# Chemical118/TREW

Hardware: AMD Instinct MI355X
Metric: Gbases/s scanned (short 5 32, 150 bp reads) (higher is better)
Workload: dtype u32

## Files before the change

include/trew_hip.h:

```cpp
#ifndef TREW_HIP_H
#define TREW_HIP_H

#include <stddef.h>
#include <stdint.h>

#ifdef __cplusplus
extern "C" {
#endif

#define TREW_HIP_ABI_VERSION 4

enum {
    TREW_MODE_SHORT = 0,
    TREW_MODE_PAIR = 1,
    TREW_MODE_LONG = 2,
    TREW_MODE_SEGMENT = 3
};

enum {
    TREW_TABLE_FORWARD_HIGH = 0,
    TREW_TABLE_FORWARD_LOW = 1,
    TREW_TABLE_BACKWARD_HIGH = 2,
    TREW_TABLE_BACKWARD_LOW = 3,
    TREW_TABLE_BOTH_HIGH = 4,
    TREW_TABLE_BOTH_LOW = 5,
    TREW_NUM_TABLES = 6
};

enum {
    TREW_FLAG_NO_FILTER = 1,
    TREW_FLAG_DEBUG_NO_EMIT = 2,
    TREW_FLAG_DEBUG_NO_KLOOP = 4,
    TREW_FLAG_DEBUG_POISON_LDS = 32,
    TREW_FLAG_DEBUG_WIDE_NO_WAIT = 128,
    TREW_FLAG_NO_TIMING = 64,
    TREW_FLAG_COMPAT_G1 = 512,
    TREW_FLAG_DEBUG_NO_JOINT = 2048,
    TREW_FLAG_DEBUG_NO_GROUP = 1024,
    TREW_FLAG_TRACK_PRESSURE = 256
};

typedef struct {
    int32_t min_mer;
    int32_t max_mer;
    double low_baseline;
    double high_baseline;
    int32_t slice_length;
    int32_t mode;
    int32_t device;
    int32_t n_slots;
    uint64_t max_batch_words;
    uint64_t max_batch_reads;
    uint32_t table_log2_slots;
    uint32_t flags;
    uint64_t max_batch_ascii_bytes;
} trew_hip_params;

typedef struct {
    const uint32_t *words;
    uint64_t n_words;
    const uint32_t *offsets;
    const uint32_t *lengths;
    uint32_t uniform_length;
    uint32_t uniform_stride;
    uint64_t n_reads;
    int32_t on_device;
    int32_t max_length;
} trew_hip_batch;

typedef struct {
    const char *bases;
    uint64_t n_bytes;
    const uint32_t *byte_offsets;
    const uint32_t *lengths;
    const uint32_t *word_offsets;
    uint32_t uniform_length;
    uint32_t reserved;
    uint64_t n_reads;
} trew_hip_ascii_batch;

typedef struct {
    int32_t k;
    int32_t table;
    uint64_t word_lo;
    uint64_t word_hi;
    uint64_t count;
} trew_hip_row;

typedef struct trew_hip_ctx trew_hip_ctx;

int trew_hip_init(const trew_hip_params *params, trew_hip_ctx **out);
void trew_hip_destroy(trew_hip_ctx *ctx);
const char *trew_hip_last_error(const trew_hip_ctx *ctx);

int trew_hip_submit(trew_hip_ctx *ctx, const trew_hip_batch *batch, int slot);
int trew_hip_submit_ascii(trew_hip_ctx *ctx, const trew_hip_ascii_batch *batch, int slot);
int trew_hip_pack_ascii(trew_hip_ctx *ctx, const trew_hip_ascii_batch *batch, uint32_t *words, uint64_t words_cap, uint64_t *n_words);
int trew_hip_wait(trew_hip_ctx *ctx, int slot);

int trew_hip_collect(trew_hip_ctx *ctx, int table, trew_hip_row *rows, uint64_t cap, uint64_t *n_rows);
int trew_hip_reset_tables(trew_hip_ctx *ctx);
int trew_hip_add_rows(trew_hip_ctx *ctx, const trew_hip_row *rows, uint64_t n_rows);

int trew_hip_collect_device(trew_hip_ctx *ctx, trew_hip_row *d_rows, uint64_t cap, uint64_t *n_rows);
int trew_hip_add_rows_device(trew_hip_ctx *ctx, const trew_hip_row *d_rows, uint64_t n_rows);
int trew_hip_merge(trew_hip_ctx *dst, trew_hip_ctx *src);
int trew_hip_add_gathered_device(trew_hip_ctx *ctx, const trew_hip_row *d_buf, uint32_t n_slices, uint32_t own_slice,
                                 uint64_t slice_rows, void *producer_stream, uint64_t *max_rows);
int trew_hip_collect_slice_device(trew_hip_ctx *ctx, trew_hip_row *d_slice, uint64_t slice_rows, void *consumer_stream, uint64_t *n_rows);

int trew_hip_table_pressure(trew_hip_ctx *ctx, uint64_t *used_slots, uint64_t *total_slots, uint64_t *spilled_rows,
                            uint64_t *spill_capacity);

#define TREW_DEBUG_COUNTERS 8
int trew_hip_debug_counters(trew_hip_ctx *ctx, uint64_t *out, int n);

int trew_hip_debug_worklist(trew_hip_ctx *ctx, int slot, uint32_t *units, uint64_t cap, uint64_t *n);

int trew_hip_segment_results(trew_hip_ctx *ctx, int slot, int32_t *k_high, int32_t *k_low,
                             uint64_t *seq_high, uint64_t *seq_low, uint64_t *seq_high_hi, uint64_t *seq_low_hi,
                             uint64_t n_reads);
int trew_hip_filter_masks(trew_hip_ctx *ctx, const trew_hip_batch *batch, uint64_t *cand, int slots_per_read);

int trew_hip_last_timing(trew_hip_ctx *ctx, int slot, float *ms_filter, float *ms_exact, uint64_t *n_flagged);

uint64_t trew_pack_words(uint64_t n_bases);
uint64_t trew_pack_reads(const char *buf, const int64_t *st, const int64_t *nd, uint64_t n_reads,
                         uint32_t *words, uint64_t words_cap, uint32_t *offsets, uint32_t *lengths);

uint64_t trew_pack_pairs(const char *buf1, const int64_t *st1, const int64_t *nd1,
                         const char *buf2, const int64_t *st2, const int64_t *nd2, uint64_t n_pairs,
                         uint32_t *words, uint64_t words_cap, uint32_t *offsets, uint32_t *lengths);

int trew_synth_short_ascii(uint64_t seed, uint64_t first_read, uint64_t n_reads, uint32_t read_len, char *out);
int trew_synth_short_device(trew_hip_ctx *ctx, uint64_t seed, uint64_t first_read, uint64_t n_reads,
                            uint32_t read_len, uint32_t *d_words);
int trew_synth_pair_ascii(uint64_t seed, uint64_t first_pair, uint64_t n_pairs, uint32_t read_len, char *out1, char *out2);
int trew_synth_pair_device(trew_hip_ctx *ctx, uint64_t seed, uint64_t first_pair, uint64_t n_pairs,
                           uint32_t read_len, uint32_t *d_words);

int trew_synth_long_lengths(uint64_t seed, uint64_t first_read, uint64_t n_reads, uint32_t *lengths);
int trew_synth_long_ascii(uint64_t seed, uint64_t first_read, uint64_t n_reads, const uint64_t *byte_offsets, char *out);
int trew_synth_long_device(trew_hip_ctx *ctx, uint64_t seed, uint64_t first_read, uint64_t n_reads,
                           const uint32_t *d_offsets, uint32_t *d_words);

int trew_hip_malloc(trew_hip_ctx *ctx, uint64_t bytes, void **d_ptr);
int trew_hip_free(trew_hip_ctx *ctx, void *d_ptr);
int trew_hip_memcpy_h2d(trew_hip_ctx *ctx, void *d_dst, const void *h_src, uint64_t bytes);
int trew_hip_memcpy_d2h(trew_hip_ctx *ctx, void *h_dst, const void *d_src, uint64_t bytes);
int trew_hip_host_alloc(trew_hip_ctx *ctx, uint64_t bytes, void **h_ptr);
int trew_hip_host_free(trew_hip_ctx *ctx, void *h_ptr);
int trew_hip_device_count(void);
int trew_hip_abi_version(void);

#ifdef __cplusplus
}
#endif
#endif
```

trew_amd/__init__.py:

```python
from . import capi
from .capi import (
    FLAG_NO_FILTER,
    FLAG_DEBUG_POISON_LDS,
    FLAG_NO_TIMING,
    FLAG_TRACK_PRESSURE,
    FLAG_COMPAT_G1,
    FLAG_DEBUG_NO_GROUP,
    FLAG_DEBUG_NO_JOINT,
    FLAG_DEBUG_WIDE_NO_WAIT,
    MODE_LONG,
    MODE_PAIR,
    MODE_SEGMENT,
    MODE_SHORT,
    TABLE_NAMES,
    TrewHip,
    TrewHipError,
    k_mer_check,
    pack_reads,
)
```

trew_amd/capi.py:

```python
from __future__ import annotations

import ctypes as C
import os

import numpy as np

_HERE = os.path.dirname(os.path.abspath(__file__))
LIB_PATH = os.environ.get("TREW_HIP_LIB") or os.path.join(_HERE, "lib", "libtrew_hip.so")

MODE_SHORT, MODE_PAIR, MODE_LONG, MODE_SEGMENT = 0, 1, 2, 3
FLAG_NO_FILTER = 1
FLAG_DEBUG_POISON_LDS = 32
FLAG_NO_TIMING = 64
FLAG_COMPAT_G1 = 512
FLAG_TRACK_PRESSURE = 256
FLAG_DEBUG_NO_JOINT = 2048
FLAG_DEBUG_NO_GROUP = 1024
FLAG_DEBUG_WIDE_NO_WAIT = 128
TABLE_NAMES = ("forward_high", "forward_low", "backward_high", "backward_low", "both_high", "both_low")

EXPORTED_SYMBOLS = (
    "trew_hip_init", "trew_hip_destroy", "trew_hip_last_error", "trew_hip_submit", "trew_hip_wait",
    "trew_hip_collect", "trew_hip_reset_tables", "trew_hip_add_rows", "trew_hip_segment_results",
    "trew_hip_filter_masks", "trew_hip_last_timing", "trew_pack_words", "trew_pack_reads",
    "trew_synth_short_ascii", "trew_synth_short_device", "trew_synth_pair_ascii", "trew_synth_pair_device",
    "trew_hip_malloc", "trew_hip_free", "trew_hip_memcpy_h2d", "trew_hip_memcpy_d2h", "trew_hip_abi_version",
    "trew_pack_pairs", "trew_hip_host_alloc", "trew_hip_host_free", "trew_hip_device_count",
    "trew_synth_long_lengths", "trew_synth_long_ascii", "trew_synth_long_device",
    "trew_hip_collect_device", "trew_hip_add_rows_device", "trew_hip_merge", "trew_hip_table_pressure",
    "trew_hip_add_gathered_device", "trew_hip_collect_slice_device", "trew_hip_debug_counters", "trew_hip_debug_worklist", "trew_hip_submit_ascii", "trew_hip_pack_ascii",
)
DEBUG_COUNTERS = ("strict_rerun", "windows_fallback", "wide_spin_timeout", "inserted", "inserted_wide", "group_punt", "group_routed", "group_target")


class Params(C.Structure):
    _fields_ = [
        ("min_mer", C.c_int32), ("max_mer", C.c_int32),
        ("low_baseline", C.c_double), ("high_baseline", C.c_double),
        ("slice_length", C.c_int32), ("mode", C.c_int32), ("device", C.c_int32), ("n_slots", C.c_int32),
        ("max_batch_words", C.c_uint64), ("max_batch_reads", C.c_uint64),
        ("table_log2_slots", C.c_uint32), ("flags", C.c_uint32),
        ("max_batch_ascii_bytes", C.c_uint64),
    ]


class Batch(C.Structure):
    _fields_ = [
        ("words", C.c_void_p), ("n_words", C.c_uint64),
        ("offsets", C.c_void_p), ("lengths", C.c_void_p),
        ("uniform_length", C.c_uint32), ("uniform_stride", C.c_uint32),
        ("n_reads", C.c_uint64), ("on_device", C.c_int32), ("max_length", C.c_int32),
    ]


class AsciiBatch(C.Structure):
    _fields_ = [
        ("bases", C.c_void_p), ("n_bytes", C.c_uint64),
        ("byte_offsets", C.c_void_p), ("lengths", C.c_void_p), ("word_offsets", C.c_void_p),
        ("uniform_length", C.c_uint32), ("reserved", C.c_uint32), ("n_reads", C.c_uint64),
    ]


class Row(C.Structure):
    _fields_ = [("k", C.c_int32), ("table", C.c_int32), ("word_lo", C.c_uint64), ("word_hi", C.c_uint64),
                ("count", C.c_uint64)]


ROW_DTYPE = np.dtype([("k", "<i4"), ("table", "<i4"), ("word_lo", "<u8"), ("word_hi", "<u8"), ("count", "<u8")])
assert ROW_DTYPE.itemsize == C.sizeof(Row)

_lib = None


def rows_to_tables(rows):
    out = {name: {} for name in TABLE_NAMES}
    if len(rows) == 0:
        return out
    for t, k, lo, hi, c in zip(rows["table"].tolist(), rows["k"].tolist(), rows["word_lo"].tolist(),
                               rows["word_hi"].tolist(), rows["count"].tolist()):
        out[TABLE_NAMES[t]][(k, (hi << 64) | lo)] = c
    return out


def tables_to_rows(tables):
    items = [(k, t, w & 0xFFFFFFFFFFFFFFFF, w >> 64, c)
             for t, name in enumerate(TABLE_NAMES) for (k, w), c in tables.get(name, {}).items()]
    return np.array(items, dtype=ROW_DTYPE) if items else np.zeros(0, dtype=ROW_DTYPE)


def load():
    global _lib
    if _lib is not None:
        return _lib
    if not os.path.exists(LIB_PATH):
        raise OSError("libtrew_hip.so is not built: run `python -c 'import __graft_entry__ as g; g.build()'`")
    lib = C.CDLL(LIB_PATH)
    vp, u64, i32 = C.c_void_p, C.c_uint64, C.c_int
    lib.trew_hip_abi_version.restype = i32
    lib.trew_hip_init.argtypes = [C.POINTER(Params), C.POINTER(vp)]
    lib.trew_hip_destroy.argtypes = [vp]
    lib.trew_hip_destroy.restype = None
    lib.trew_hip_last_error.argtypes = [vp]
    lib.trew_hip_last_error.restype = C.c_char_p
    lib.trew_hip_submit.argtypes = [vp, C.POINTER(Batch), i32]
    lib.trew_hip_wait.argtypes = [vp, i32]
    lib.trew_hip_submit_ascii.argtypes = [vp, C.POINTER(AsciiBatch), i32]
    lib.trew_hip_pack_ascii.argtypes = [vp, C.POINTER(AsciiBatch), vp, u64, C.POINTER(u64)]
    lib.trew_hip_collect.argtypes = [vp, i32, C.POINTER(Row), u64, C.POINTER(u64)]
    lib.trew_hip_reset_tables.argtypes = [vp]
    lib.trew_hip_add_rows.argtypes = [vp, C.POINTER(Row), u64]
    lib.trew_hip_collect_device.argtypes = [vp, vp, u64, C.POINTER(u64)]
    lib.trew_hip_add_rows_device.argtypes = [vp, vp, u64]
    lib.trew_hip_merge.argtypes = [vp, vp]
    lib.trew_hip_add_gathered_device.argtypes = [vp, vp, C.c_uint32, C.c_uint32, u64, vp, C.POINTER(u64)]
    lib.trew_hip_collect_slice_device.argtypes = [vp, vp, u64, vp, C.POINTER(u64)]
    lib.trew_hip_debug_counters.argtypes = [vp, C.POINTER(u64), i32]
    lib.trew_hip_debug_worklist.argtypes = [vp, i32, vp, u64, C.POINTER(u64)]
    lib.trew_hip_table_pressure.argtypes = [vp, C.POINTER(u64), C.POINTER(u64), C.POINTER(u64), C.POINTER(u64)]
    lib.trew_hip_segment_results.argtypes = [vp, i32, vp, vp, vp, vp, vp, vp, u64]
    lib.trew_hip_filter_masks.argtypes = [vp, C.POINTER(Batch), vp, i32]
    lib.trew_hip_last_timing.argtypes = [vp, i32, C.POINTER(C.c_float), C.POINTER(C.c_float), C.POINTER(u64)]
    lib.trew_pack_words.argtypes = [u64]
    lib.trew_pack_words.restype = u64
    lib.trew_pack_reads.argtypes = [C.c_char_p, vp, vp, u64, vp, u64, vp, vp]
    lib.trew_pack_reads.restype = u64
    lib.trew_synth_short_ascii.argtypes = [u64, u64, u64, C.c_uint32, vp]
    lib.trew_synth_short_device.argtypes = [vp, u64, u64, u64, C.c_uint32, vp]
    lib.trew_synth_pair_ascii.argtypes = [u64, u64, u64, C.c_uint32, vp, vp]
    lib.trew_synth_pair_device.argtypes = [vp, u64, u64, u64, C.c_uint32, vp]
    lib.trew_synth_long_lengths.argtypes = [u64, u64, u64, vp]
    lib.trew_synth_long_ascii.argtypes = [u64, u64, u64, vp, vp]
    lib.trew_synth_long_device.argtypes = [vp, u64, u64, u64, vp, vp]
    lib.trew_hip_malloc.argtypes = [vp, u64, C.POINTER(vp)]
    lib.trew_hip_free.argtypes = [vp, vp]
    lib.trew_hip_memcpy_h2d.argtypes = [vp, vp, vp, u64]
    lib.trew_hip_memcpy_d2h.argtypes = [vp, vp, vp, u64]
    _lib = lib
    return lib


class TrewHipError(RuntimeError):
    pass


def pack_reads(reads):
    lib = load()
    reads = [r.encode() if isinstance(r, str) else bytes(r) for r in reads]
    n = len(reads)
    st = np.zeros(n, dtype=np.int64)
    nd = np.zeros(n, dtype=np.int64)
    pos = 0
    for i, r in enumerate(reads):
        st[i] = pos
        nd[i] = pos + len(r) - 1
        pos += len(r) + 1
    buf = b"\n".join(reads) + b"\n"
    cap = int(sum(lib.trew_pack_words(len(r)) for r in reads)) + 8
    words = np.zeros(cap, dtype=np.uint32)
    offsets = np.zeros(max(n, 1), dtype=np.uint32)
    lengths = np.zeros(max(n, 1), dtype=np.uint32)
    w = lib.trew_pack_reads(buf, st.ctypes.data, nd.ctypes.data, n, words.ctypes.data, cap, offsets.ctypes.data,
                            lengths.ctypes.data)
    if w == 2 ** 64 - 1:
        raise TrewHipError("trew_pack_reads: buffer too small")
    return words[: int(w)], offsets[:n], lengths[:n]


def synth_short_ascii(seed, first_read, n_reads, read_len):
    lib = load()
# ... 276 lines not shown
```

trew_amd/csrc/kernels/prefilter.inc:

```


template <int NW>
__device__ __forceinline__ void prefix_parity(const u32 (&f)[NW], u32 (&P)[NW]) {
    u32 carry = 0, prev_top = 0;
#pragma unroll
    for (int j = 0; j < NW; j++) {
        u32 x = f[j];
        x ^= x << 1;
        x ^= x << 2;
        x ^= x << 4;
        x ^= x << 8;
        x ^= x << 16;
        x ^= carry;
        P[j] = (x << 1) | prev_top;
        prev_top = x >> 31;
        carry = 0u - prev_top;
    }
}

template <>
__device__ __forceinline__ void prefix_parity<3>(const u32 (&f)[3], u32 (&P)[3]) {
    u64 x = ((u64) f[1] << 32) | f[0];
    x ^= x << 1;
    x ^= x << 2;
    x ^= x << 4;
    x ^= x << 8;
    x ^= x << 16;
    x ^= x << 32;
    u32 y = f[2];
    y ^= y << 1;
    y ^= y << 2;
    y ^= y << 4;
    y ^= y << 8;
    y ^= y << 16;
    const u32 top = (u32) (x >> 63);
    y ^= 0u - top;
    const u64 e = x << 1;
    P[0] = (u32) e;
    P[1] = (u32) (e >> 32);
    P[2] = (y << 1) | top;
}

__device__ __forceinline__ u32 xor_and(u32 x, u32 y, u32 m) { return __builtin_amdgcn_bitop3_b32(x, y, m, 0x28); }

__device__ __forceinline__ u64 all_k_mask(int kmin, int kmax) {
    if (kmax < kmin) return 0;
    u64 hi = kmax >= 64 ? ~0ull : ((1ull << kmax) - 1ull);
    u64 lo = (1ull << (kmin - 1)) - 1ull;
    return hi & ~lo;
}

template <int NW, int WS>
__device__ __forceinline__ u32 shr_word(const u32 (&x)[NW], int j, u32 bs) {
    const u32 lo = (j + WS < NW) ? x[j + WS < NW ? j + WS : 0] : 0u;
    const u32 hi = (j + WS + 1 < NW) ? x[j + WS + 1 < NW ? j + WS + 1 : 0] : 0u;
    return alignbit(hi, lo, bs);
}

template <int NW, int WS, int NWW>
__device__ __forceinline__ void filter_k(const u32 (&P1)[NW], const u32 (&P2)[NW], const u32 (&P3)[NW],
                                         const u32 (&v1)[NW], u32 (&V)[NW], int k, float lowf, u32 &cand_lo, u32 &cand_hi) {
    const u32 bs = (u32) k & 31u;
    u32 c01 = 0, c10 = 0, c11 = 0, count = 0;
#pragma unroll
    for (int j = 0; j < NWW; j++) {
        const u32 F1 = P1[j] ^ shr_word<NW, WS>(P1, j, bs), F2 = P2[j] ^ shr_word<NW, WS>(P2, j, bs);
        const u32 v = V[j];
        const u32 a1 = v & F1;
        const u32 a11 = a1 & F2;
        count += __popc(v);
        c11 += __popc(a11);
        c10 += __popc(a1 ^ a11);
        c01 += __popc((v ^ a1) & F2);
    }
    const u32 c00 = count - c01 - c10 - c11;
    const u32 m4 = max(max(c00, c01), max(c10, c11));
    const float thr = (float) count * lowf;
    const bool pass4 = (float) m4 > thr;
    bool pass = pass4;
    const bool first = (cand_lo | cand_hi) == 0;
    if (__any(pass4 && first)) {
        u32 c001 = 0, c010 = 0, c011 = 0, c100 = 0, c101 = 0, c110 = 0, c111 = 0;
#pragma unroll
        for (int j = 0; j < NWW; j++) {
            const u32 F1 = P1[j] ^ shr_word<NW, WS>(P1, j, bs), F2 = P2[j] ^ shr_word<NW, WS>(P2, j, bs);
            const u32 F3 = P3[j] ^ shr_word<NW, WS>(P3, j, bs);
            const u32 v = V[j];
            const u32 a1 = v & F1, a0 = v ^ a1;
            const u32 a11 = a1 & F2, a10 = a1 ^ a11, a01 = a0 & F2, a00 = a0 ^ a01;
            const u32 b111 = a11 & F3, b101 = a10 & F3, b011 = a01 & F3, b001 = a00 & F3;
            c111 += __popc(b111);
            c110 += __popc(a11 ^ b111);
            c101 += __popc(b101);
            c100 += __popc(a10 ^ b101);
            c011 += __popc(b011);
            c010 += __popc(a01 ^ b011);
            c001 += __popc(b001);
        }
        const u32 c000 = count - c001 - c010 - c011 - c100 - c101 - c110 - c111;
        const u32 m8 = max(max(max(c000, c001), max(c010, c011)), max(max(c100, c101), max(c110, c111)));
        pass = first ? ((float) m8 > thr) : pass4;
    }
    if (k <= 32)
        cand_lo |= pass ? (1u << ((k - 1) & 31)) : 0u;
    else
        cand_hi |= pass ? (1u << ((k - 33) & 31)) : 0u;
#pragma unroll
    for (int j = 0; j < NWW; j++) V[j] &= shr_word<NW, WS>(v1, j, bs);
}

template <int NW, int WS, int NWW>
struct FilterRange {
    static __device__ __forceinline__ void run(const u32 (&P1)[NW], const u32 (&P2)[NW], const u32 (&P3)[NW], const u32 (&v1)[NW],
                                               u32 (&V)[NW], int klo, int khi, int max_seg, float lowf, u32 &clo, u32 &chi) {
        int a = max_seg + 2 - 32 * NWW, b = max_seg + 1 - 32 * (NWW - 1);
        if (NWW == NW) a = klo;
        a = a < klo ? klo : a;
        b = b > khi ? khi : b;
        for (int k = a; k <= b; k++) filter_k<NW, WS, NWW>(P1, P2, P3, v1, V, k, lowf, clo, chi);
        FilterRange<NW, WS, NWW - 1>::run(P1, P2, P3, v1, V, klo, khi, max_seg, lowf, clo, chi);
    }
};
template <int NW, int WS>
struct FilterRange<NW, WS, 0> {
    static __device__ __forceinline__ void run(const u32 (&)[NW], const u32 (&)[NW], const u32 (&)[NW], const u32 (&)[NW], u32 (&)[NW],
                                               int, int, int, float, u32 &, u32 &) {}
};

template <int NW>
__device__ __forceinline__ u64 filter_segment(const u32 (&lo)[NW], const u32 (&hi)[NW], const u32 (&nm)[NW], int L,
                                              int kmin, int kmax, int gmin, int gmax, int max_seg, float lowf) {
    u32 v1[NW], P1[NW], P2[NW], P3[NW], V[NW];
    {
        u32 f1[NW], f2[NW], f3[NW];
#pragma unroll
        for (int j = 0; j < NW; j++) {
            int bits = L - 32 * j;
            u32 lm = bits >= 32 ? 0xffffffffu : (bits <= 0 ? 0u : ((1u << bits) - 1u));
            v1[j] = ~nm[j] & lm;
            f1[j] = lo[j] & v1[j];
            f2[j] = hi[j] & v1[j];
            f3[j] = f1[j] & f2[j];
            V[j] = v1[j];
        }
        prefix_parity<NW>(f1, P1);
        prefix_parity<NW>(f2, P2);
        prefix_parity<NW>(f3, P3);
    }
    for (int t = 1; t < gmin && t < 32; t++) {
#pragma unroll
        for (int j = 0; j < NW; j++) V[j] &= shr_word<NW, 0>(v1, j, (u32) t);
    }
    for (int t = 32; t < gmin && t < 64; t++) {
#pragma unroll
        for (int j = 0; j < NW; j++) V[j] &= shr_word<NW, 1>(v1, j, (u32) t & 31u);
    }
    u32 clo = 0, chi = 0;
    const int g31 = gmax < 31 ? gmax : 31;
    if (NW <= 5) {
        FilterRange<NW, 0, NW>::run(P1, P2, P3, v1, V, gmin, g31, max_seg, lowf, clo, chi);
        FilterRange<NW, 1, NW>::run(P1, P2, P3, v1, V, gmin > 32 ? gmin : 32, gmax < 63 ? gmax : 63, max_seg, lowf, clo, chi);
        FilterRange<NW, 2, NW>::run(P1, P2, P3, v1, V, gmin > 64 ? gmin : 64, gmax, max_seg, lowf, clo, chi);
    } else {
        for (int k = gmin; k <= g31; k++) filter_k<NW, 0, NW>(P1, P2, P3, v1, V, k, lowf, clo, chi);
        for (int k = gmin > 32 ? gmin : 32; k <= (gmax < 63 ? gmax : 63); k++) filter_k<NW, 1, NW>(P1, P2, P3, v1, V, k, lowf, clo, chi);
        for (int k = gmin > 64 ? gmin : 64; k <= gmax; k++) filter_k<NW, 2, NW>(P1, P2, P3, v1, V, k, lowf, clo, chi);
    }
    return ((((u64) chi) << 32) | clo) & all_k_mask(kmin, kmax);
}


template <int NW, int WS, int NWW, bool SUBSET = false>
__device__ __forceinline__ u64 filter_k_uni(const u32 (&P1)[NW], const u32 (&P2)[NW], const u32 (&P3)[NW], int L, int k,
                                            const int2 th, u64 hasm) {
    const u32 bs = (u32) k & 31u;
    const int W = SUBSET ? 32 * NWW : L - k + 1;
    const int lastbits = W - 32 * (NWW - 1);
    const u32 wm = SUBSET ? 0xffffffffu : (1u << (lastbits & 31)) - 1u;
    u32 F1[NWW], F2[NWW];
    u32 c1x = 0, cx1 = 0, c11 = 0;
#pragma unroll
    for (int j = 0; j < NWW; j++) {
        F1[j] = P1[j] ^ shr_word<NW, WS>(P1, j, bs);
        F2[j] = P2[j] ^ shr_word<NW, WS>(P2, j, bs);
        if (j == NWW - 1 && !SUBSET) {
            F1[j] &= wm;
            F2[j] &= wm;
            asm volatile("" : "+v"(F1[j]), "+v"(F2[j]));
        }
        c1x = bcnt_acc(F1[j], c1x);
        cx1 = bcnt_acc(F2[j], cx1);
        c11 = bcnt_acc(F1[j] & F2[j], c11);
    }
    const u32 c10 = c1x - c11, c01 = cx1 - c11;
    const u32 m3 = max(max(c10, c01), c11);
    const int t = (int) (c1x + c01);
    const u64 p4 = __ballot(m3 >= (u32) th.x) | __ballot(t <= th.y);
    u64 pm = p4;
    if (p4 & ~hasm) {
        u32 c001 = 0, c010 = 0, c011 = 0, c100 = 0, c101 = 0, c110 = 0, c111 = 0;
#pragma unroll
        for (int j = 0; j < NWW; j++) {
            const u32 F3 = P3[j] ^ shr_word<NW, WS>(P3, j, bs);
            const u32 v = j == NWW - 1 ? wm : 0xffffffffu;
            const u32 a11 = F1[j] & F2[j], a10 = F1[j] & ~F2[j], a01 = ~F1[j] & F2[j], a00 = v & ~(F1[j] | F2[j]);
            const u32 b111 = a11 & F3, b101 = a10 & F3, b011 = a01 & F3, b001 = a00 & F3;
            c111 += __popc(b111);
            c110 += __popc(a11 ^ b111);
            c101 += __popc(b101);
            c100 += __popc(a10 ^ b101);
            c011 += __popc(b011);
            c010 += __popc(a01 ^ b011);
            c001 += __popc(b001);
        }
        const u32 c000 = (u32) W - c001 - c010 - c011 - c100 - c101 - c110 - c111;
        const u32 m8 = max(max(max(c000, c001), max(c010, c011)), max(max(c100, c101), max(c110, c111)));
        const u64 p8 = __ballot(m8 >= (u32) th.x);
        pm = (p4 & hasm) | (p8 & ~hasm);
    }
    return pm;
}

__device__ __forceinline__ u64 container64(const u32 (&P)[3], int s) {
    const bool big = s >= 32;
    const u32 lo = alignbit(big ? P[2] : P[1], big ? P[1] : P[0], (u32) s & 31u);
    const u32 hi = alignbit(big ? 0u : P[2], big ? P[2] : P[1], (u32) s & 31u);
    return ((u64) hi << 32) | lo;
}

__device__ __forceinline__ u64 filter_k_uni_q(const u32 (&P1)[3], const u32 (&P2)[3], const u32 (&P3)[3], u64 Q1, u64 Q2, int s, int L, int k,
                                              const int2 th, u64 hasm) {
    const int W = L - k + 1;
    const u32 sh = (u32) (k - s);
#ifndef TREW_AB_NO_Q
// ... 149 lines not shown
                }
            }
        }
        {
            const int s = L > 63 ? L - 63 : 0;
            int a = L - 63, b = L - 31;
            a = a < gmin ? gmin : a;
            b = b > gmax ? gmax : b;
            if (a <= b) {
                const u64 Q1 = container64(P1, s), Q2 = container64(P2, s);
                int2 th_next = thr_row[a - 1];
                for (int k = a; k <= b; k++) {
                    const int2 th = th_next;
                    th_next = thr_row[k];
                    note(filter_k_uni_q(P1, P2, P3, Q1, Q2, s, L, k, th, vd.hasm), k);
                }
            }
        }
        if (slow) {
            FilterRangeUni<NW, 0, 1, true>::run(P1, P2, P3, gmin, g31, L, kmin, kmax, thr_row, dbg, vd);
            FilterRangeUni<NW, 1, 1, true>::run(P1, P2, P3, gmin > 32 ? gmin : 32, gmax < 63 ? gmax : 63, L, kmin, kmax, thr_row, dbg, vd);
            FilterRangeUni<NW, 2, 1, true>::run(P1, P2, P3, gmin > 64 ? gmin : 64, gmax, L, kmin, kmax, thr_row, dbg, vd);
        } else {
            FilterRangeUni<NW, 0, 1, false>::run(P1, P2, P3, gmin, g31, L, kmin, kmax, thr_row, false, vd);
            FilterRangeUni<NW, 1, 1, false>::run(P1, P2, P3, gmin > 32 ? gmin : 32, gmax < 63 ? gmax : 63, L, kmin, kmax, thr_row, false, vd);
            FilterRangeUni<NW, 2, 1, false>::run(P1, P2, P3, gmin > 64 ? gmin : 64, gmax, L, kmin, kmax, thr_row, false, vd);
        }
        if (!slow) vd.flagm = vd.hasm;
    } else {
        if (slow) {
            FilterRangeUni<NW, 0, NW, true>::run(P1, P2, P3, gmin, g31, L, kmin, kmax, thr_row, dbg, vd);
            FilterRangeUni<NW, 1, NW, true>::run(P1, P2, P3, gmin > 32 ? gmin : 32, gmax < 63 ? gmax : 63, L, kmin, kmax, thr_row, dbg, vd);
            FilterRangeUni<NW, 2, NW, true>::run(P1, P2, P3, gmin > 64 ? gmin : 64, gmax, L, kmin, kmax, thr_row, dbg, vd);
        } else {
            FilterRangeUni<NW, 0, NW, false>::run(P1, P2, P3, gmin, g31, L, kmin, kmax, thr_row, false, vd);
            FilterRangeUni<NW, 1, NW, false>::run(P1, P2, P3, gmin > 32 ? gmin : 32, gmax < 63 ? gmax : 63, L, kmin, kmax, thr_row, false, vd);
            FilterRangeUni<NW, 2, NW, false>::run(P1, P2, P3, gmin > 64 ? gmin : 64, gmax, L, kmin, kmax, thr_row, false, vd);
            vd.flagm = vd.hasm;
        }
    }
}

struct HalvesP {
    u32 P1[3], P2[3];
};
__device__ __forceinline__ void halves_prefix(const u32 (&lo)[3], const u32 (&hi)[3], int L, HalvesP &o) {
    u32 f1[3], f2[3];
#pragma unroll
    for (int j = 0; j < 3; j++) {
        const int bits = L - 32 * j;
        const u32 lm = bits >= 32 ? 0xffffffffu : (bits <= 0 ? 0u : ((1u << bits) - 1u));
        f1[j] = lo[j] & lm;
        f2[j] = hi[j] & lm;
    }
    prefix_parity<3>(f1, o.P1);
    prefix_parity<3>(f2, o.P2);
}
__device__ __forceinline__ u32 bcnt_acc_s(u32 x, int acc) {
    u32 d;
    asm("v_bcnt_u32_b32 %0, %1, %2" : "=v"(d) : "v"(x), "s"(acc));
    return d;
}
__device__ __forceinline__ void halves_signs(u32 F1a, u32 F2a, u32 F1b, u32 F2b, int n2, int n1, int K, u32 &x, u32 &t) {
    u32 a = bcnt_acc_s(F1a, n2);
    u32 b = bcnt_acc_s(F2a, n2);
    u32 c = bcnt_acc_s(F1a & F2a, n1);
    a = bcnt_acc(F1b, a);
    b = bcnt_acc(F2b, b);
    c = bcnt_acc(F1b & F2b, c);
    const u32 p = a - c, q = b - c;
    x = __builtin_amdgcn_bitop3_b32(p, q, c, 0x80);
    t = a + q + (u32) K;
}
__device__ __forceinline__ u64 halves_verdict(u32 xA, u32 tA, u32 xB, u32 tB) {
    const u32 y = __builtin_amdgcn_bitop3_b32(xA, xB, tA, 0x40);
    const u32 z = __builtin_amdgcn_bitop3_b32(y, tB, tB, 0x30);
    return __ballot((int) z >= 0);
}
struct Thr8 {
    int4 a, b;
};
__device__ __forceinline__ Thr8 load_thr8(const int4 *p) {
    typedef int v8i __attribute__((ext_vector_type(8)));
    typedef const __attribute__((address_space(4))) v8i *cptr;
    const v8i v = *(cptr) (unsigned long long) p;
    Thr8 o;
    o.a = make_int4(v[0], v[1], v[2], v[3]);
    o.b = make_int4(v[4], v[5], v[6], v[7]);
    return o;
}
__device__ __forceinline__ int4 load_thr4(const int4 *p) {
    typedef int v4i __attribute__((ext_vector_type(4)));
    typedef const __attribute__((address_space(4))) v4i *cptr;
    const v4i v = *(cptr) (unsigned long long) p;
    return make_int4(v.x, v.y, v.z, v.w);
}

__device__ __forceinline__ const int4 *joint_thresholds(const int2 *thr_tab) { return (const int4 *) (thr_tab + kThrRows * kThrRow); }

__device__ __forceinline__ u64 filter_halves_uni(const HalvesP &A, const HalvesP &Bh, int L, int klo, int khi, const int4 *__restrict__ thr_row,
                                                 const u32 *wm_tab) {
    u64 trig = 0;
    int k = klo;
    const int4 *tp = thr_row + (klo - 1);
    {
        int b = L - 64;
        b = b > khi ? khi : b;
        auto probe = [&](u32 bs, const int4 t) __attribute__((always_inline)) -> u64 {
            u32 xA, tA, xB, tB;
            halves_signs(A.P1[0] ^ alignbit(A.P1[1], A.P1[0], bs), A.P2[0] ^ alignbit(A.P2[1], A.P2[0], bs), A.P1[1] ^ alignbit(A.P1[2], A.P1[1], bs),
                         A.P2[1] ^ alignbit(A.P2[2], A.P2[1], bs), t.x, t.y, t.z, xA, tA);
            halves_signs(Bh.P1[0] ^ alignbit(Bh.P1[1], Bh.P1[0], bs), Bh.P2[0] ^ alignbit(Bh.P2[1], Bh.P2[0], bs), Bh.P1[1] ^ alignbit(Bh.P1[2], Bh.P1[1], bs),
                         Bh.P2[1] ^ alignbit(Bh.P2[2], Bh.P2[1], bs), t.x, t.y, t.z, xB, tB);
            return halves_verdict(xA, tA, xB, tB);
        };
        for (; k + 1 <= b; k += 2, tp += 2) {
            const Thr8 t8 = load_thr8(tp);
            trig |= probe((u32) k, t8.a);
            trig |= probe((u32) k + 1u, t8.b);
        }
        if (k <= b) {
            trig |= probe((u32) k, load_thr4(tp));
            k++, tp++;
        }
    }
    if (k <= khi) {
        const int b = khi;
        const int s = L > 63 ? L - 63 : 0;
        const u64 QA1 = container64(A.P1, s), QA2 = container64(A.P2, s), QB1 = container64(Bh.P1, s), QB2 = container64(Bh.P2, s);
        u32 sh = (u32) (k - s);
        typedef const __attribute__((address_space(3))) u32 *lds_u32;
        u32 wa = (u32) (unsigned long long) (lds_u32) wm_tab + 4u * (u32) (63 - (L - k));
        asm volatile("" : "+v"(wa));
        auto probe = [&](u32 shk, u32 wmk, const int4 t) __attribute__((always_inline)) -> u64 {
            const u64 SA1 = QA1 >> shk, SA2 = QA2 >> shk, SB1 = QB1 >> shk, SB2 = QB2 >> shk;
            const u32 gA1 = xor_and(A.P1[1], (u32) (SA1 >> 32), wmk), gA2 = xor_and(A.P2[1], (u32) (SA2 >> 32), wmk);
            const u32 gB1 = xor_and(Bh.P1[1], (u32) (SB1 >> 32), wmk), gB2 = xor_and(Bh.P2[1], (u32) (SB2 >> 32), wmk);
            u32 xA, tA, xB, tB;
            halves_signs(A.P1[0] ^ (u32) SA1, A.P2[0] ^ (u32) SA2, gA1, gA2, t.x, t.y, t.z, xA, tA);
            halves_signs(Bh.P1[0] ^ (u32) SB1, Bh.P2[0] ^ (u32) SB2, gB1, gB2, t.x, t.y, t.z, xB, tB);
            return halves_verdict(xA, tA, xB, tB);
        };
        for (; k + 1 <= b; k += 2, sh += 2u, wa += 8u, tp += 2) {
            const Thr8 t8 = load_thr8(tp);
            const u32 wm0 = *(lds_u32) (unsigned long long) wa, wm1 = *(lds_u32) (unsigned long long) (wa + 4u);
            trig |= probe(sh, wm0, t8.a);
            trig |= probe(sh + 1u, wm1, t8.b);
        }
        if (k <= b) trig |= probe(sh, *(lds_u32) (unsigned long long) wa, load_thr4(tp));
    }
    return trig;
}

constexpr u32 kFilterThreads = TREW_FILTER_THREADS;
constexpr u32 kStage = kFilterThreads == 256 ? 1024 : 192;
constexpr u32 kDefer = 2 * kFilterThreads;

template <int NW>
#ifndef TREW_FILTER3_WAVES
#define TREW_FILTER3_WAVES 6
#endif
#ifndef TREW_FILTER5_WAVES
#define TREW_FILTER5_WAVES 6
#endif
__global__ __launch_bounds__(kFilterThreads, (NW <= 3 ? TREW_FILTER3_WAVES : (NW == 5 ? TREW_FILTER5_WAVES : 1))) void filter_kernel(DevParams P, DevBatch B, u32 *wl, u32 *wl_count, u32 wl_cap,
                                                                u64 *dbg_masks, int dbg_slots, int max_seg, u32 *diag,
                                                                const int2 *__restrict__ thr_tab) {
#ifdef TREW_AB_FILTER_PRIO
    __builtin_amdgcn_s_setprio(TREW_AB_FILTER_PRIO);
#endif
    __shared__ u32 stage[kStage];
    __shared__ u32 stage_n, flush_base;
    __shared__ u32 defer_n;
    u32 defer_seen = 0;
    if (threadIdx.x == 0) stage_n = 0;
    __syncthreads();
    auto flush = [&]() __attribute__((always_inline)) {
        const u32 n = stage_n;
        if (n) {
            if (threadIdx.x == 0) flush_base = atomicAdd(wl_count, n);
            __syncthreads();
            const u32 fb = flush_base;
            for (u32 i = threadIdx.x; i < n; i += blockDim.x) {
                if (fb + i < wl_cap)
                    wl[fb + i] = stage[i];
                else
                    atomicAdd(&diag[kDiagWorklistDrop], 1u);
            }
            __syncthreads();
            if (threadIdx.x == 0) stage_n = 0;
        }
        __syncthreads();
    };
    auto append = [&](bool flag, u32 unit) __attribute__((always_inline)) {
        const u64 bal = __ballot(flag);
        if (bal) {
            const u32 lane = lane_id();
            const int leader = __ffsll((long long) bal) - 1;
            u32 sb = 0;
            if ((int) lane == leader) sb = atomicAdd(&stage_n, (u32) __popcll(bal));
            sb = __shfl(sb, leader);
            if (flag) stage[sb + (u32) __popcll(bal & ((1ull << lane) - 1ull))] = unit;
        }
        __syncthreads();
        const bool full = stage_n > kStage - kFilterThreads;
        defer_seen = defer_n;
        __syncthreads();
        if (full) flush();
    };
    const int nslots = mode_slots(P.mode);
    const int gmax_run = (P.flags & TREW_FLAG_DEBUG_NO_KLOOP) ? P.min_mer - 1 : P.max_mer;
    auto general = [&](u64 unit, bool active) __attribute__((always_inline)) -> u64 {
        ReadRef rd[2];
        rd[0].w = B.words;
        rd[0].len = 0;
        rd[0].nw = 0;
        rd[1] = rd[0];
        if (active) {
            if (P.mode == TREW_MODE_PAIR) {
                rd[0] = get_read(B, 2 * unit);
                rd[1] = get_read(B, 2 * unit + 1);
            } else {
                rd[0] = get_read(B, unit);
            }
        }
        u64 any = 0;
#pragma unroll
        for (int slot = 0; slot < kMaxSlots; slot++) {
            if (slot < nslots) {
                u64 mask = 0;
                Segment sg = get_segment(P.mode, slot, rd[0].len, rd[1].len, P.min_mer, P.max_mer, P.slice_len);
                const bool ok = active && sg.valid && sg.len <= (u32) (32 * NW - 1);
                if (__any(ok)) {
                    u32 lo[NW], hi[NW], nm[NW];
                    const ReadRef &r = sg.mate ? rd[1] : rd[0];
                    if (ok) {
                        load_planes<NW>(r, sg.start, lo, hi, nm);
                    } else {
#pragma unroll
                        for (int j = 0; j < NW; j++) {
                            lo[j] = hi[j] = 0;
                            nm[j] = 0xffffffffu;
                        }
                    }
                    u64 m;
                    if (P.flags & TREW_FLAG_NO_FILTER)
                        m = all_k_mask(sg.kmin, sg.kmax);
                    else
                        m = filter_segment<NW>(lo, hi, nm, ok ? (int) sg.len : 0, sg.kmin, sg.kmax, P.min_mer, gmax_run, max_seg, P.lowf);
                    mask = ok ? m : 0ull;
                }
                if (active && sg.valid && sg.len > (u32) (32 * NW - 1)) mask = all_k_mask(sg.kmin, sg.kmax);
                any |= mask;
                if (dbg_masks && active && slot < dbg_slots) dbg_masks[unit * (u64) dbg_slots + slot] = mask;
            }
        }
        return any;
    };

    __shared__ u32 defer[kDefer];
    __shared__ unsigned char defer_kind[kDefer];
    __shared__ u32 wm_tab[34];
    if (threadIdx.x < 34) wm_tab[threadIdx.x] = threadIdx.x < 32 ? 0xffffffffu >> threadIdx.x : 0u;
    const u32 UL = B.uniform_length;
    const bool uni = NW <= 5 && UL != 0 && thr_tab != nullptr && P.mode != TREW_MODE_LONG && !(P.flags & TREW_FLAG_NO_FILTER);
    if (threadIdx.x == 0) defer_n = 0;
    __syncthreads();
    __shared__ u32 next_chunk[2];
    constexpr u32 kChunkShards = 8;
    const u32 my_shard = blockIdx.x & (kChunkShards - 1u);
    auto shard_ctr = [&](u32 sh) __attribute__((always_inline)) { return wl_count + 32u + 32u * sh + kChunkCounterWord; };
    u64 chunk = blockIdx.x;
    u32 round = 0;
    for (;;) {
        const bool more = chunk * kFilterThreads < B.n_units;
        if (more) {
            const u64 unit = chunk * kFilterThreads + threadIdx.x;
            const bool active = unit < B.n_units;
            u32 nxt = 0;
#ifndef TREW_AB_STATIC_CHUNKS
            if (threadIdx.x == 0) nxt = gridDim.x + kChunkShards * atomicAdd(shard_ctr(my_shard), 1u) + my_shard;
#else
            nxt = (u32) chunk + gridDim.x;
#endif
            u64 any = 0;
            bool dfr = active, dfr_n = false;
            if constexpr (NW <= 5) {
                if (uni) {
                    ReadRef rd[2];
                    rd[0].w = B.words;
                    rd[0].len = 0;
                    rd[0].nw = 0;
                    rd[1] = rd[0];
                    if (active) {
                        if (P.mode == TREW_MODE_PAIR) {
                            rd[0] = get_read(B, 2 * unit);
                            rd[1] = get_read(B, 2 * unit + 1);
                        } else {
                            rd[0] = get_read(B, unit);
                        }
                    }
                    dfr = false;
                    int slot0 = 0;
#ifndef TREW_AB_NO_JOINT
                    if constexpr (NW == 3) {
                        const int n_halves = P.mode == TREW_MODE_PAIR ? 4 : (P.mode == TREW_MODE_SHORT ? 2 : 0);
                        for (; slot0 + 1 < n_halves && !dbg_masks && !(P.flags & TREW_FLAG_DEBUG_NO_JOINT); slot0 += 2) {
                            const Segment sA = get_segment(P.mode, slot0, UL, UL, P.min_mer, P.max_mer, P.slice_len);
                            const Segment sB = get_segment(P.mode, slot0 + 1, UL, UL, P.min_mer, P.max_mer, P.slice_len);
                            const int L = rfl_i((int) sA.len);
                            const int klo = rfl_i(sA.kmin > P.min_mer ? sA.kmin : P.min_mer), khi = rfl_i(sA.kmax < gmax_run ? sA.kmax : gmax_run);
                            const bool uneq = sB.len == sA.len + 1u;
                            if (!(sA.valid && sB.valid && (sA.len == sB.len || uneq) && sA.len <= 95u && sA.kmin == sB.kmin && sA.kmax == sB.kmax &&
                                  klo >= L + 1 - kUniSubsetMax && khi <= L - 32 && klo <= 31))
                                break;
                            u32 loA[3], hiA[3], nmA[3], loB[3], hiB[3], nmB[3];
                            load_planes<3>(sA.mate ? rd[1] : rd[0], sA.start, loA, hiA, nmA);
                            load_planes<3>(sB.mate ? rd[1] : rd[0], sB.start, loB, hiB, nmB);
                            u32 anyn = 0;
#pragma unroll
                            for (int j = 0; j < 3; j++) {
                                const int bits = L - 32 * j, bitsB = (int) sB.len - 32 * j;
                                const u32 lm = bits >= 32 ? 0xffffffffu : (bits <= 0 ? 0u : ((1u << bits) - 1u));
                                const u32 lmB = bitsB >= 32 ? 0xffffffffu : (bitsB <= 0 ? 0u : ((1u << bitsB) - 1u));
                                anyn |= (nmA[j] & lm) | (nmB[j] & lmB);
                            }
                            dfr = dfr || (active && anyn != 0);
                            dfr_n = dfr_n || (active && anyn != 0);
                            HalvesP hA, hB;
                            halves_prefix(loA, hiA, L, hA);
                            halves_prefix(loB, hiB, L, hB);
                            const u64 trig = filter_halves_uni(hA, hB, L, klo, khi, joint_thresholds(thr_tab) + (uneq ? 2 + slot0 / 2 : slot0 / 2) * kThrRow, wm_tab);
                            dfr = dfr || (active && any == 0 && ((trig >> lane_id()) & 1ull) != 0);
                        }
                    }
#endif
                    for (int slot = slot0; slot < nslots; slot++) {
                        const Segment sg = get_segment(P.mode, slot, UL, UL, P.min_mer, P.max_mer, P.slice_len);
                        if (!sg.valid) continue;
                        if (sg.len > (u32) (32 * NW - 1)) {
                            dfr = dfr || active;
                            continue;
                        }
                        u32 lo[NW], hi[NW], nm[NW];
                        const ReadRef r = sg.mate ? rd[1] : rd[0];
                        load_planes<NW>(r, sg.start, lo, hi, nm);
                        u32 anyn = 0;
#pragma unroll
                        for (int j = 0; j < NW; j++) {
                            const int bits = (int) sg.len - 32 * j;
                            const u32 lm = bits >= 32 ? 0xffffffffu : (bits <= 0 ? 0u : ((1u << bits) - 1u));
                            anyn |= nm[j] & lm;
                        }
                        UniVerdict vd;
                        filter_segment_uni<NW>(lo, hi, (int) sg.len, sg.kmin, sg.kmax, P.min_mer, gmax_run, thr_tab + slot * kThrRow, dbg_masks != nullptr, vd);
                        dfr = dfr || (active && anyn != 0);
                        dfr_n = dfr_n || (active && anyn != 0);
                        any |= (vd.flagm >> lane_id()) & 1ull;
                        if (dbg_masks && active && anyn == 0 && slot < dbg_slots)
                            dbg_masks[unit * (u64) dbg_slots + slot] = ((((u64) vd.chi) << 32) | vd.clo) & all_k_mask(sg.kmin, sg.kmax);
                    }
                }
            }
            {
                const u64 bal = __ballot(dfr);
                if (bal) {
                    const u32 lane = lane_id();
                    const int leader = __ffsll((long long) bal) - 1;
                    u32 sb = 0;
                    if ((int) lane == leader) sb = atomicAdd(&defer_n, (u32) __popcll(bal));
                    sb = __shfl(sb, leader);
                    if (dfr) {
                        const u32 at = sb + (u32) __popcll(bal & ((1ull << lane) - 1ull));
                        defer[at] = (u32) unit;
                        defer_kind[at] = dfr_n ? 1 : 0;
                    }
                }
            }
            if (threadIdx.x == 0) next_chunk[round & 1u] = nxt;
            append(active && !dfr && any != 0, (u32) unit);
            chunk = next_chunk[round & 1u];
#ifndef TREW_AB_STATIC_CHUNKS
            if (chunk * kFilterThreads >= B.n_units) {
                __syncthreads();
                if (threadIdx.x == 0) {
                    u64 c = chunk;
                    for (u32 att = 1; att < kChunkShards && c * kFilterThreads >= B.n_units; att++) {
                        const u32 sh = (my_shard + att) & (kChunkShards - 1u);
                        c = (u64) gridDim.x + (u64) kChunkShards * atomicAdd(shard_ctr(sh), 1u) + sh;
                    }
                    next_chunk[round & 1u] = (u32) (c < 0xffffffffull ? c : 0xffffffffull);
                }
                __syncthreads();
                chunk = next_chunk[round & 1u];
                __syncthreads();
            }
#endif
            round++;
        }
        const u32 dn = defer_seen;
        if (dn >= kFilterThreads || (!more && dn > 0u)) {
            const u32 take = dn < kFilterThreads ? dn : kFilterThreads;
            const u32 at = dn - take;
            const bool active2 = threadIdx.x < take;
            const u32 unit2 = active2 ? defer[at + threadIdx.x] : 0u;
            const bool n2 = active2 && defer_kind[at + threadIdx.x] != 0;
            __syncthreads();
            if (threadIdx.x == 0) defer_n = at;
            const u64 any2 = general(unit2, active2);
            append(active2 && any2 != 0 && !n2, unit2);
            append(active2 && any2 != 0 && n2, unit2);
        } else if (!more) {
            break;
        }
    }
    flush();
}
```

Measured before the change: 1905.

## Add specialized uniform-length drain path for deferred filter units

Adds a specialized deferred-unit filter for uniform-length short and paired reads with three-word segments. It processes both halves of a pair together using prefix-parity planes, a shared-memory table of count thresholds, and wave-level early exit once every lane is flagged. This replaces the general per-unit filter in the drain phase. The goal is to cut the cost of re-filtering deferred units, in exchange for extra LDS, more kernel code and register pressure, and a second filter path whose results must match the general one. Debug and A/B macros plus a flag that disables the path are added.

```diff
diff --git a/include/trew_hip.h b/include/trew_hip.h
--- a/include/trew_hip.h
+++ b/include/trew_hip.h
@@ -36,6 +36,7 @@
     TREW_FLAG_NO_TIMING = 64,
     TREW_FLAG_COMPAT_G1 = 512,
     TREW_FLAG_DEBUG_NO_JOINT = 2048,
+    TREW_FLAG_DEBUG_NO_UNI_DRAIN = 4096,
     TREW_FLAG_DEBUG_NO_GROUP = 1024,
     TREW_FLAG_TRACK_PRESSURE = 256
 };
diff --git a/trew_amd/__init__.py b/trew_amd/__init__.py
--- a/trew_amd/__init__.py
+++ b/trew_amd/__init__.py
@@ -7,6 +7,7 @@
     FLAG_COMPAT_G1,
     FLAG_DEBUG_NO_GROUP,
     FLAG_DEBUG_NO_JOINT,
+    FLAG_DEBUG_NO_UNI_DRAIN,
     FLAG_DEBUG_WIDE_NO_WAIT,
     MODE_LONG,
     MODE_PAIR,
diff --git a/trew_amd/capi.py b/trew_amd/capi.py
--- a/trew_amd/capi.py
+++ b/trew_amd/capi.py
@@ -15,6 +15,7 @@
 FLAG_COMPAT_G1 = 512
 FLAG_TRACK_PRESSURE = 256
 FLAG_DEBUG_NO_JOINT = 2048
+FLAG_DEBUG_NO_UNI_DRAIN = 4096
 FLAG_DEBUG_NO_GROUP = 1024
 FLAG_DEBUG_WIDE_NO_WAIT = 128
 TABLE_NAMES = ("forward_high", "forward_low", "backward_high", "backward_low", "both_high", "both_low")
diff --git a/trew_amd/csrc/kernels/prefilter.inc b/trew_amd/csrc/kernels/prefilter.inc
--- a/trew_amd/csrc/kernels/prefilter.inc
+++ b/trew_amd/csrc/kernels/prefilter.inc
@@ -79,7 +79,11 @@
     const bool pass4 = (float) m4 > thr;
     bool pass = pass4;
     const bool first = (cand_lo | cand_hi) == 0;
+#ifdef TREW_AB_SKIP_DRAIN8
+    if (false) {
+#else
     if (__any(pass4 && first)) {
+#endif
         u32 c001 = 0, c010 = 0, c011 = 0, c100 = 0, c101 = 0, c110 = 0, c111 = 0;
 #pragma unroll
         for (int j = 0; j < NWW; j++) {
@@ -535,6 +539,183 @@
     return trig;
 }
 
+constexpr int kCntThr = 97;
+__device__ __forceinline__ int4 count_thresholds(int c, float lowf) {
+    const float prod = __fmul_rn((float) c, lowf);
+    const int ithr = (int) floorf(prod) + 1;
+    return make_int4(-2 * ithr, -ithr, 4 * ithr - c - 1, ithr);
+}
+
+struct DrainHalf {
+    u32 P1[3], P2[3], P3[3];
+    u32 V[3];
+};
+__device__ __forceinline__ void drain_half_init(const u32 (&lo)[3], const u32 (&hi)[3], const u32 (&nm)[3], int L, bool active, DrainHalf &h) {
+    u32 f1[3], f2[3], f3[3];
+#pragma unroll
+    for (int j = 0; j < 3; j++) {
+        const int bits = L - 32 * j;
+        const u32 lm = bits >= 32 ? 0xffffffffu : (bits <= 0 ? 0u : ((1u << bits) - 1u));
+        h.V[j] = active ? ~nm[j] & lm : 0u;
+        f1[j] = lo[j] & lm;
+        f2[j] = hi[j] & lm;
+        f3[j] = f1[j] & f2[j];
+    }
+    prefix_parity<3>(f1, h.P1);
+    prefix_parity<3>(f2, h.P2);
+    prefix_parity<3>(f3, h.P3);
+}
+__device__ __forceinline__ void drain_v_step3(u32 (&V)[3]) {
+    V[0] &= alignbit(V[1], V[0], 1u);
+    V[1] &= alignbit(V[2], V[1], 1u);
+    V[2] &= V[2] >> 1;
+}
+template <int N>
+__device__ __forceinline__ int drain_signs(const u32 (&F1)[N], const u32 (&F2)[N], const int4 th) {
+    u32 a = (u32) th.x, b = (u32) th.x, c = (u32) th.y;
+#pragma unroll
+    for (int j = 0; j < N; j++) {
+        a = bcnt_acc(F1[j], a);
+        b = bcnt_acc(F2[j], b);
+        c = bcnt_acc(F1[j] & F2[j], c);
+    }
+    const u32 p = a - c, q = b - c;
+    const u32 t = a + q + (u32) th.z;
+    return (int) __builtin_amdgcn_bitop3_b32(__builtin_amdgcn_bitop3_b32(p, q, c, 0x80), t, t, 0x30);
+}
+template <int N>
+__device__ __forceinline__ bool drain_pass8(const u32 (&F1)[N], const u32 (&F2)[N], const u32 (&F3)[N], const u32 (&V)[N], u32 count, int ithr) {
+    u32 c001 = 0, c010 = 0, c011 = 0, c100 = 0, c101 = 0, c110 = 0, c111 = 0;
+#pragma unroll
+    for (int j = 0; j < N; j++) {
+        const u32 a11 = F1[j] & F2[j], a10 = F1[j] & ~F2[j], a01 = ~F1[j] & F2[j], a00 = V[j] & ~(F1[j] | F2[j]);
+        const u32 b111 = a11 & F3[j], b101 = a10 & F3[j], b011 = a01 & F3[j], b001 = a00 & F3[j];
+        c111 += __popc(b111);
+        c110 += __popc(a11 ^ b111);
+        c101 += __popc(b101);
+        c100 += __popc(a10 ^ b101);
+        c011 += __popc(b011);
+        c010 += __popc(a01 ^ b011);
+        c001 += __popc(b001);
+    }
+    const u32 c000 = count - c001 - c010 - c011 - c100 - c101 - c110 - c111;
+    const u32 m8 = max(max(max(c000, c001), max(c010, c011)), max(max(c100, c101), max(c110, c111)));
+    return (int) m8 >= ithr;
+}
+
+__device__ __forceinline__ bool drain_uni_applies(const DevParams &P, u32 UL, int gmax_run) {
+    const int n_halves = P.mode == TREW_MODE_PAIR ? 4 : (P.mode == TREW_MODE_SHORT ? 2 : 0);
+    if (n_halves == 0) return false;
+    for (int slot = n_halves; slot < mode_slots(P.mode); slot++)
+        if (get_segment(P.mode, slot, UL, UL, P.min_mer, P.max_mer, P.slice_len).valid) return false;
+    for (int p = 0; p < n_halves; p += 2) {
+        const Segment a = get_segment(P.mode, p, UL, UL, P.min_mer, P.max_mer, P.slice_len);
+        const Segment b = get_segment(P.mode, p + 1, UL, UL, P.min_mer, P.max_mer, P.slice_len);
+        const int la = (int) a.len, lb = (int) b.len, lmin = la < lb ? la : lb, lmax = la < lb ? lb : la;
+        const int khi = a.kmax < gmax_run ? a.kmax : gmax_run;
+        if (!(a.valid && b.valid && a.kmin == b.kmin && a.kmax == b.kmax && lmax <= 95 && lmax - lmin <= 1 && a.kmin >= 1 && khi <= lmin)) return false;
+    }
+    return true;
+}
+
+__device__ __forceinline__ bool filter_deferred_uni(const DevParams &P, const DevBatch &B, u64 unit, bool active, int gmax_run,
+                                                    const int4 *cnt_thr) {
+    const u32 UL = B.uniform_length;
+    ReadRef rd[2];
+    rd[0].w = B.words;
+    rd[0].len = 0;
+    rd[0].nw = 0;
+    rd[1] = rd[0];
+    if (active) {
+        if (P.mode == TREW_MODE_PAIR) {
+            rd[0] = get_read(B, 2 * unit);
+            rd[1] = get_read(B, 2 * unit + 1);
+        } else {
+            rd[0] = get_read(B, unit);
+        }
+    }
+    const u64 actm = __ballot(active);
+    u64 flag = 0;
+    const int n_halves = P.mode == TREW_MODE_PAIR ? 4 : 2;
+    for (int p = 0; p < n_halves && flag != actm; p += 2) {
+        const Segment sA = get_segment(P.mode, p, UL, UL, P.min_mer, P.max_mer, P.slice_len);
+        const Segment sB = get_segment(P.mode, p + 1, UL, UL, P.min_mer, P.max_mer, P.slice_len);
+        const int LA = rfl_i((int) sA.len), LB = rfl_i((int) sB.len), Lmax = LA < LB ? LB : LA;
+        const int klo = rfl_i(sA.kmin > P.min_mer ? sA.kmin : P.min_mer), khi = rfl_i(sA.kmax < gmax_run ? sA.kmax : gmax_run);
+        DrainHalf A, Bh;
+        {
+            u32 lo[3], hi[3], nm[3];
+            load_planes<3>(sA.mate ? rd[1] : rd[0], sA.start, lo, hi, nm);
+            drain_half_init(lo, hi, nm, LA, active, A);
+            load_planes<3>(sB.mate ? rd[1] : rd[0], sB.start, lo, hi, nm);
+            drain_half_init(lo, hi, nm, LB, active, Bh);
+        }
+        for (int t = 1; t < klo; t++) {
+            drain_v_step3(A.V);
+            drain_v_step3(Bh.V);
+        }
+        int k = klo;
+        {
+            const int b = khi < Lmax - 64 ? khi : Lmax - 64;
+            auto half3 = [&](const DrainHalf &h, u32 bs) __attribute__((always_inline)) -> u64 {
+                const u32 cnt = bcnt_acc(h.V[2], bcnt_acc(h.V[1], __popc(h.V[0])));
+                const int4 th = cnt_thr[cnt];
+                u32 F1[3], F2[3];
+#pragma unroll
+                for (int j = 0; j < 3; j++) {
+                    F1[j] = xor_and(h.P1[j], alignbit(j < 2 ? h.P1[j < 2 ? j + 1 : 0] : 0u, h.P1[j], bs), h.V[j]);
+                    F2[j] = xor_and(h.P2[j], alignbit(j < 2 ? h.P2[j < 2 ? j + 1 : 0] : 0u, h.P2[j], bs), h.V[j]);
+                }
+                const u64 p4 = __ballot(drain_signs<3>(F1, F2, th) >= 0);
+                u64 p8 = 0;
+                if (p4 & ~flag) {
+                    u32 F3[3];
+#pragma unroll
+                    for (int j = 0; j < 3; j++) F3[j] = h.P3[j] ^ alignbit(j < 2 ? h.P3[j < 2 ? j + 1 : 0] : 0u, h.P3[j], bs);
+                    p8 = __ballot(drain_pass8<3>(F1, F2, F3, h.V, cnt, th.w));
+                }
+                return p8;
+            };
+            for (; k <= b && flag != actm; k++) {
+                flag |= half3(A, (u32) k);
+                flag |= half3(Bh, (u32) k);
+                drain_v_step3(A.V);
+                drain_v_step3(Bh.V);
+            }
+        }
+        if (k <= khi && flag != actm) {
+            const int oA = LA > 63 ? LA - 63 : 0, oB = LB > 63 ? LB - 63 : 0;
+            const u64 QA1 = container64(A.P1, oA), QA2 = container64(A.P2, oA), QB1 = container64(Bh.P1, oB), QB2 = container64(Bh.P2, oB);
+            u64 VA = ((u64) A.V[1] << 32) | A.V[0], VB = ((u64) Bh.V[1] << 32) | Bh.V[0];
+            auto half2 = [&](const DrainHalf &h, u64 Q1, u64 Q2, u64 V, int s) __attribute__((always_inline)) -> u64 {
+                const u32 v0 = (u32) V, v1 = (u32) (V >> 32);
+                const u32 cnt = bcnt_acc(v1, __popc(v0));
+                const int4 th = cnt_thr[cnt];
+                const u32 sh = (u32) (k - s);
+                const u64 S1 = Q1 >> sh, S2 = Q2 >> sh;
+                const u32 F1[2] = {xor_and(h.P1[0], (u32) S1, v0), xor_and(h.P1[1], (u32) (S1 >> 32), v1)};
+                const u32 F2[2] = {xor_and(h.P2[0], (u32) S2, v0), xor_and(h.P2[1], (u32) (S2 >> 32), v1)};
+                const u64 p4 = __ballot(drain_signs<2>(F1, F2, th) >= 0);
+                u64 p8 = 0;
+                if (p4 & ~flag) {
+                    const u64 S3 = container64(h.P3, s) >> sh;
+                    const u32 F3[2] = {h.P3[0] ^ (u32) S3, h.P3[1] ^ (u32) (S3 >> 32)};
+                    const u32 Vw[2] = {v0, v1};
+                    p8 = __ballot(drain_pass8<2>(F1, F2, F3, Vw, cnt, th.w));
+                }
+                return p8;
+            };
+            for (; k <= khi && flag != actm; k++) {
+                flag |= half2(A, QA1, QA2, VA, oA);
+                flag |= half2(Bh, QB1, QB2, VB, oB);
+                VA &= VA >> 1;
+                VB &= VB >> 1;
+            }
+        }
+    }
+    return (flag >> lane_id()) & 1ull;
+}
+
 constexpr u32 kFilterThreads = TREW_FILTER_THREADS;
 constexpr u32 kStage = kFilterThreads == 256 ? 1024 : 192;
 constexpr u32 kDefer = 2 * kFilterThreads;
@@ -645,8 +826,11 @@
     __shared__ unsigned char defer_kind[kDefer];
     __shared__ u32 wm_tab[34];
     if (threadIdx.x < 34) wm_tab[threadIdx.x] = threadIdx.x < 32 ? 0xffffffffu >> threadIdx.x : 0u;
+    __shared__ int4 cnt_thr[kCntThr];
+    for (u32 i = threadIdx.x; i < (u32) kCntThr; i += blockDim.x) cnt_thr[i] = count_thresholds((int) i, P.lowf);
     const u32 UL = B.uniform_length;
     const bool uni = NW <= 5 && UL != 0 && thr_tab != nullptr && P.mode != TREW_MODE_LONG && !(P.flags & TREW_FLAG_NO_FILTER);
+    const bool uni_drain = NW == 3 && uni && !dbg_masks && !(P.flags & TREW_FLAG_DEBUG_NO_UNI_DRAIN) && drain_uni_applies(P, UL, gmax_run);
     if (threadIdx.x == 0) defer_n = 0;
     __syncthreads();
     __shared__ u32 next_chunk[2];
@@ -790,7 +974,14 @@
             const bool n2 = active2 && defer_kind[at + threadIdx.x] != 0;
             __syncthreads();
             if (threadIdx.x == 0) defer_n = at;
-            const u64 any2 = general(unit2, active2);
+#ifndef TREW_AB_SKIP_DRAIN
+            const u64 any2 = uni_drain ? (u64) filter_deferred_uni(P, B, unit2, active2, gmax_run, cnt_thr) : general(unit2, active2);
+#else
+            u64 any2 = 0;
+            u32 keep = unit2;
+            asm volatile("" : "+v"(keep), "+v"(any2));
+            (void) keep;
+#endif
             append(active2 && any2 != 0 && !n2, unit2);
             append(active2 && any2 != 0 && n2, unit2);
         } else if (!more) {
```

After: 1991, median of 6. 4.5% higher.
